# iammcy/BFLC-demo

Measured on NVIDIA H100. Metric: federated_rounds_per_sec, higher is better.
Workload: dtype mxfp8

## Files before the change

bflc_demo_b200/csrc/kernels/mlp_round_sm100.cu:

```cuda
#include <cuda_bf16.h>

#include <algorithm>
#include <cstdlib>
#include <cstring>
#include <type_traits>

#include "bflc_kernels.h"
#include "epi_common.cuh"
#include "fed_admit.cuh"
#include "launch.cuh"
#include "sm100_ptx.cuh"
#include "wgmma.cuh"

namespace bflc {

namespace {

using epi::kStgLd;
using epi::stage_put;
using epi::stage_get;
using epi::col_sum32;
using epi::st_sw128;
__device__ __forceinline__ uint32_t pack2(float a, float b) { return epi::pack_bf16x2(a, b); }

constexpr int kBM = 128, kBN = 64, kStages = 5;
constexpr int kABytes = kBM * 128, kBBytes = kBN * 128, kStageBytes = kABytes + kBBytes;
constexpr int kTileBytes = kStages * kStageBytes;
constexpr int kBarBytes = 512;
constexpr int kEpiWarps = 8;
constexpr int kEpiThreads = kEpiWarps * 32;
constexpr int kStgAll = kEpiWarps * 32 * kStgLd * 4;
constexpr int kBiasFloats = 320;
constexpr int kXchFloats = 4 * 2 * 128;
constexpr int kAccPitch = kBN + 4;
constexpr int kAccBytes = kBM * kAccPitch * 4;
constexpr int kSmemTotal = kTileBytes + kBarBytes + kStgAll + (kBiasFloats + kXchFloats) * 4 + kAccBytes + 1024;
static_assert(kSmemTotal <= 227 * 1024, "shared memory budget");
constexpr int kEpiT0 = 128;
constexpr int kProducerWarp = 4 + kEpiWarps;
constexpr int kThreads = kEpiT0 + kEpiThreads + 128;
constexpr int kProducerRegs = 40, kMmaRegs = 184, kEpiRegs = 144;
static_assert(kProducerRegs + kMmaRegs + 2 * kEpiRegs <= 4 * 128, "register file");
enum Role : int { kRoleProducer = 0, kRoleMma = 1, kRoleEpi = 2 };
constexpr int kGrid = 32;

constexpr int kOffH = 0;
constexpr int kOffW2K = 64 * 1024;
constexpr int kOffW2MN = 96 * 1024;
constexpr int kOffDL = 104 * 1024;
static_assert(kOffDL + 16384 <= kTileBytes, "chain smem layout");
constexpr int kChainH = 256;
constexpr int kDefaultPlan = 4;
constexpr int kCluster = 4;

enum EpiMode : int { E_BIAS_RELU_BF16 = 0, E_XENT = 1, E_F32 = 2, E_MASK_COLSUM_BF16 = 3,
                     E_OPT = 4 };

struct Maps {
  CUtensorMap x_k, w1_k, h_k, w2_k, dl_mn, h_mn, dl_k, w2_mn, dh_mn, x_mn;
};

struct Args {
  int B, steps, in_dim, hidden, n_classes, ncp;
  int chain;
  int epiopt;
  unsigned long long* dbg;
  const unsigned int* x_ready;
  const unsigned int* round_seq;
// ... 82 lines not shown
}

__device__ __forceinline__ void produce_tile(const Job& j, uint8_t* smem, uint64_t* full_bar, uint64_t* empty_bar,
                                             Pipe& pp) {
  const uint32_t a_bytes = static_cast<uint32_t>(j.bm) * 128u;
  for (int i = 0; i < j.n_kb; ++i, ++pp.it) {
    const int s = pp.it % kStages;
    const uint32_t ph = (pp.it / kStages) & 1;
    ptx::mbar_wait(&empty_bar[s], ph ^ 1);
    uint8_t* sa = smem + s * kStageBytes;
    uint8_t* sb = sa + kABytes;
    if (ptx::elect_one()) {
      ptx::mbar_expect_tx(&full_bar[s], a_bytes + kBBytes);
      if (!j.a_mn) {
        ptx::tma_load_3d(sa, j.ta, &full_bar[s], j.a_c0 + i * 64, j.a_c1, 0);
      } else {
        ptx::tma_load_3d(sa, j.ta, &full_bar[s], j.a_c0, j.a_c1 + i * 64, 0);
        if (j.bm == kBM) ptx::tma_load_3d(sa + 64 * 128, j.ta, &full_bar[s], j.a_c0 + 64, j.a_c1 + i * 64, 0);
      }
      if (!j.b_mn)
        ptx::tma_load_3d(sb, j.tb, &full_bar[s], j.b_c0 + i * 64, j.b_c1, 0);
      else
        ptx::tma_load_3d(sb, j.tb, &full_bar[s], j.b_c0, j.b_c1 + i * 64, 0);
    }
    __syncwarp();
  }
}

__device__ __forceinline__ int lane128(int r) { return r; }
__device__ __forceinline__ int lane128_hi(int r) { return 64 + r; }
// ... 364 lines not shown
  }
  if (stampit) j.dbg[j.dbg_slot + 1] = globaltimer_ns();
}

__device__ __forceinline__ uint32_t pos_mask8(const uint4 u) {
  const uint32_t wds[4] = {u.x, u.y, u.z, u.w};
  uint32_t m = 0u;
#pragma unroll
  for (int e = 0; e < 4; ++e) {
    m |= (((wds[e] & 0xFFFFu) != 0u && (wds[e] & 0x8000u) == 0u) ? 1u : 0u) << (e * 2);
    m |= (((wds[e] >> 16) != 0u && (wds[e] & 0x80000000u) == 0u) ? 1u : 0u) << (e * 2 + 1);
  }
  return m;
}

template <bool FP8>
__device__ __forceinline__ uint32_t fwd1_epilogue_x(const Job& j, const Args& a, uint8_t* smem, const ChainBars& cb,
                                                    int q, int half, int lane, uint64_t* accum_bar,
                                                    const wg::AccTile& at, float* stg, float* sbias, Pipe& pp,
                                                    uint32_t par, int slice) {
  const int et = threadIdx.x - kEpiT0;
  if (et < kBN) sbias[et] = __ldcg(j.bias + j.n0 + et);
  epi_bar();
  const int rl = q * 32 + lane, row_base = j.m0 + q * 32;
  const bool row_ok = row_base + lane < j.M;
  const int cr = lane >> 3, cg = (lane & 7) * 4, nc = j.n0 + half * 32;
  const bool stampit = j.dbg != nullptr && blockIdx.x == 0 && threadIdx.x == kEpiT0;
  ptx::mbar_wait(accum_bar, pp.tile & 1);
  ++pp.tile;
  if (stampit) j.dbg[j.dbg_slot] = globaltimer_ns();
  float v[32];
  {
    uint32_t r[32];
    wg::acc_ld32(at, (static_cast<uint32_t>(q * 32) << 16) + half * 32, r);
#pragma unroll
    for (int k = 0; k < 32; ++k) v[k] = fmaxf(__uint_as_float(r[k]) + sbias[half * 32 + k], 0.f);
  }
  uint4 hv[4];
  if (FP8) {
    uint32_t w[8];
    const int e = epi::mx8_quant32(v, w);
#pragma unroll
    for (int i = 0; i < 4; ++i) {
      const uint2 lo = epi::mx8_dq4(w[2 * i], e), hi = epi::mx8_dq4(w[2 * i + 1], e);
      hv[i] = make_uint4(lo.x, lo.y, hi.x, hi.y);
    }
  } else {
#pragma unroll
    for (int jj = 0; jj < 4; ++jj)
      hv[jj] = make_uint4(pack2(v[8 * jj], v[8 * jj + 1]), pack2(v[8 * jj + 2], v[8 * jj + 3]),
                          pack2(v[8 * jj + 4], v[8 * jj + 5]), pack2(v[8 * jj + 6], v[8 * jj + 7]));
  }
  uint32_t mk = 0u;
#pragma unroll
  for (int jj = 0; jj < 4; ++jj) {
    if (!row_ok) hv[jj] = make_uint4(0u, 0u, 0u, 0u);
    mk |= pos_mask8(hv[jj]) << (jj * 8);
  }
  stage_put(stg, lane, v);
  uint8_t* hs = smem + kOffH + slice * 16384;
#pragma unroll
  for (int jj = 0; jj < 4; ++jj) st_sw128(hs, rl, half * 4 + jj, hv[jj]);
  ptx::fence_proxy_async_smem();
  epi_bar();
  if (threadIdx.x == kEpiT0) {
    const uint32_t hxa = ptx::smem_u32(cb.hx);
    ptx::mbar_expect_tx(cb.hx, (kCluster - 1) * 16384);
    ptx::mbar_wait_cluster(cb.ring_free, par);
    for (uint32_t r = 1; r < kCluster; ++r) {
      const uint32_t peer = (slice + r) % kCluster;
      ptx::bulk_s2cluster(ptx::mapa(ptx::smem_u32(hs), peer), hs, 16384, ptx::mapa(hxa, peer));
    }
  }
  if (stampit) j.dbg[1] = globaltimer_ns();
  __syncwarp();
#pragma unroll
  for (int it = 0; it < 8; ++it) {
    const int rr = it * 4 + cr, rw = row_base + rr;
    if (rw >= j.M) continue;
    const float4 x = *reinterpret_cast<const float4*>(stg + rr * kStgLd + cg);
    *reinterpret_cast<uint2*>(a.h + static_cast<long long>(rw) * j.ldd + nc + cg) =
        make_uint2(pack2(x.x, x.y), pack2(x.z, x.w));
  }
  __syncwarp();
  if (stampit) j.dbg[j.dbg_slot + 1] = globaltimer_ns();
  return mk;
}

__device__ __forceinline__ void chain_produce(const Maps& maps, uint8_t* smem, const ChainBars& cb, int m0,
                                              int slice, bool with_h) {
  if (ptx::elect_one()) {
    ptx::mbar_expect_tx(cb.w2k, 32768);
    if (with_h) ptx::mbar_expect_tx(cb.h, 65536);
    ptx::mbar_expect_tx(cb.w2mn, 8192);
    if (with_h) {
#pragma unroll
      for (int kb = 0; kb < 4; ++kb)
        ptx::tma_load_3d(smem + kOffH + kb * 16384, &maps.h_k, cb.h, kb * 64, m0, 0);
    }
#pragma unroll
    for (int kb = 0; kb < 4; ++kb)
      ptx::tma_load_3d(smem + kOffW2K + kb * 8192, &maps.w2_k, cb.w2k, kb * 64, 0, 0);
    ptx::tma_load_3d(smem + kOffW2MN, &maps.w2_mn, cb.w2mn, slice * 64, 0, 0);
  }
  __syncwarp();
}

__device__ __forceinline__ void chain_mma(uint8_t* smem, const ChainBars& cb, const wg::AccTile& at, uint32_t par,
                                          bool fused) {
  const uint32_t base = ptx::smem_u32(smem);
  ptx::mbar_wait(cb.w2k, par);
  if (fused) {
    ptx::mbar_wait_cluster(cb.hx, par);
    ptx::fence_proxy_async_smem();
  } else {
    ptx::mbar_wait(cb.h, par);
  }
  float l0[32], l1[32];
  wg::zero(l0);
  wg::zero(l1);
  const uint32_t ha = base + kOffH, wb = base + kOffW2K;
  wg::fence();
#pragma unroll
  for (uint32_t kb = 0; kb < 4; ++kb)
#pragma unroll
    for (uint32_t k = 0; k < 4; ++k) {
      const uint64_t bd = wg::desc(wb + kb * 8192u + k * 32u, 16);
      wg::mma_bf16<64, 0, 0>(l0, wg::desc(ha + kb * 16384u + k * 32u, 16), bd, (kb > 0 || k > 0) ? 1u : 0u);
      wg::mma_bf16<64, 0, 0>(l1, wg::desc(ha + kb * 16384u + 8192u + k * 32u, 16), bd, (kb > 0 || k > 0) ? 1u : 0u);
    }
  wg::commit();
  wg::wait<0>();
  wg::reg_fence(l0);
  wg::reg_fence(l1);
  wg::acc_put<64>(at, 0, l0, lane128);
  wg::acc_put<64>(at, 0, l1, lane128_hi);
  ptx::mbar_arrive(cb.acc_l);
  ptx::mbar_wait(cb.w2mn, par);
  ptx::mbar_wait(cb.dl_ready, par);
  wg::zero(l0);
  wg::zero(l1);
  wg::fence();
#pragma unroll
  for (uint32_t k = 0; k < 4; ++k) {
    const uint64_t bd = wg::desc(base + kOffW2MN + k * 2048u, 8192);
    wg::mma_bf16<64, 0, 1>(l0, wg::desc(base + kOffDL + k * 32u, 16), bd, k > 0);
    wg::mma_bf16<64, 0, 1>(l1, wg::desc(base + kOffDL + 8192u + k * 32u, 16), bd, k > 0);
  }
  wg::commit();
  wg::wait<0>();
  wg::reg_fence(l0);
  wg::reg_fence(l1);
  wg::acc_put<64>(at, 0, l0, lane128);
  wg::acc_put<64>(at, 0, l1, lane128_hi);
  ptx::mbar_arrive(cb.acc_dh);
}

__device__ __forceinline__ void chain_epilogue(const Args& a, uint8_t* smem, const ChainBars& cb,
                                               const wg::AccTile& at, int q, int half, int lane, float* stg,
                                               float* sb, float* xch, uint32_t par, int m0, int r0, int slice,
                                               unsigned long long* dbg, bool fused, uint32_t mk_fused) {
  auto stampc = [&](int slot) {
    if (dbg != nullptr && blockIdx.x == 0 && threadIdx.x == kEpiT0) dbg[slot] = globaltimer_ns();
  };
  const int rl = q * 32 + lane;
  const int row = m0 + rl;
  const bool row_ok = row < a.B;
  const int32_t label = row_ok ? __ldg(a.labels + r0 + row) : -1;
  const int C = a.n_classes;
  {
    const int et = threadIdx.x - kEpiT0;
    sb[et] = __ldcg(a.b1 + et);
    if (et < 64) sb[kChainH + et] = et < C ? __ldcg(a.b2 + et) : 0.f;
    epi_bar();
  }
  const uint32_t taddr = static_cast<uint32_t>(q * 32) << 16;
  float* xmax = xch + half * 128;            const float* omax = xch + (1 - half) * 128;
  float* xidx = xch + 256 + half * 128;      const float* oidx = xch + 256 + (1 - half) * 128;
  float* xzl = xch + 512 + half * 128;       const float* ozl = xch + 512 + (1 - half) * 128;
  float* xsum = xch + 768 + half * 128;      const float* osum = xch + 768 + (1 - half) * 128;

  uint32_t mk = mk_fused;
  if (!fused) {
    ptx::mbar_wait(cb.h, par);
    stampc(6);
    const uint8_t* hs = smem + kOffH;
    const int c = 2 * slice + half;
#pragma unroll
    for (int jj = 0; jj < 4; ++jj) mk |= pos_mask8(epi::ld_sw128(hs + (c >> 1) * 16384, rl, (c & 1) * 4 + jj)) << (jj * 8);
  } else if (dbg != nullptr && blockIdx.x == 0 && threadIdx.x == kEpiT0) {
    ptx::mbar_wait_cluster(cb.hx, par);
    stampc(6);
  }
  stampc(7);

  ptx::mbar_wait(cb.acc_l, par);
  stampc(8);
  {
    float z[32];
    {
      uint32_t ra[32];
      wg::acc_ld32(at, taddr + half * 32, ra);
#pragma unroll
      for (int k = 0; k < 32; ++k) z[k] = __uint_as_float(ra[k]) + sb[kChainH + half * 32 + k];
    }
    const int nb = half * 32;
    float pm[4] = {-INFINITY, -INFINITY, -INFINITY, -INFINITY};
    int pi[4] = {-1, -1, -1, -1};
    float zlab = 0.f;
#pragma unroll
    for (int k = 0; k < 32; ++k) {
      if (nb + k < C) {
        if (z[k] > pm[k & 3]) { pm[k & 3] = z[k]; pi[k & 3] = nb + k; }
        if (nb + k == label) zlab = z[k];
      }
    }
    float vmax = pm[0];
    int amax = pi[0];
#pragma unroll
    for (int jq = 1; jq < 4; ++jq)
      if (pm[jq] > vmax || (pm[jq] == vmax && pi[jq] >= 0 && pi[jq] < amax)) { vmax = pm[jq]; amax = pi[jq]; }
    xmax[rl] = vmax; xidx[rl] = __int_as_float(amax); xzl[rl] = zlab;
    epi_bar();
    {
      const float ov = omax[rl];
      const int oi = __float_as_int(oidx[rl]);
      const bool take = half == 0 ? (ov > vmax) : (ov >= vmax && oi >= 0);
      if (take) { vmax = ov; amax = oi; }
      zlab += ozl[rl];
    }
    stampc(12);
    float ps[4] = {0.f, 0.f, 0.f, 0.f};
#pragma unroll
    for (int k = 0; k < 32; ++k) {
      z[k] = nb + k < C ? __expf(z[k] - vmax) : 0.f;
      ps[k & 3] += z[k];
    }
    const float psum = (ps[0] + ps[1]) + (ps[2] + ps[3]);
    xsum[rl] = psum;
    epi_bar();
    const float sum = psum + osum[rl];
    const float inv = 1.f / sum;
    const float gs = 1.f / static_cast<float>(a.B);
    const bool do_colsum = slice == 1, do_global = slice == 2, do_loss = slice == 3 && half == 0;
    uint8_t* dls = smem + kOffDL;
    {
      float v[32];
#pragma unroll
      for (int k = 0; k < 32; ++k)
        v[k] = (nb + k < C && row_ok) ? (z[k] * inv - (nb + k == label ? 1.f : 0.f)) * gs : 0.f;
#pragma unroll
      for (int jj = 0; jj < 4; ++jj) {
        const uint4 u = make_uint4(pack2(v[8 * jj], v[8 * jj + 1]), pack2(v[8 * jj + 2], v[8 * jj + 3]),
                                   pack2(v[8 * jj + 4], v[8 * jj + 5]), pack2(v[8 * jj + 6], v[8 * jj + 7]));
        st_sw128(dls, rl, half * 4 + jj, u);
      }
      if (do_colsum) {
        stage_put(stg, lane, v);
        __syncwarp();
        const float tot = col_sum32(stg, lane, 32);
        if (nb + lane < C) atomicAdd(a.gb2 + nb + lane, tot);
        __syncwarp();
      }
    }
    stampc(13);
    ptx::fence_proxy_async_smem();
    ptx::mbar_arrive(cb.dl_ready);
    stampc(14);
    __syncwarp();
    if (do_global) {
#pragma unroll
      for (int it = 0; it < 4; ++it) {
        const int rt = q * 32 + it * 8 + (lane >> 2), ch = half * 4 + (lane & 3);
        const uint4 u = epi::ld_sw128(dls, rt, ch);
        if (m0 + rt < a.B && ch * 8 < a.ncp)
          *reinterpret_cast<uint4*>(a.dlogits + static_cast<long long>(m0 + rt) * a.ncp + ch * 8) = u;
      }
    }
    if (do_loss) {
      float loss = row_ok ? (__logf(sum) + vmax - zlab) : 0.f;
      const bool hit = row_ok && (amax == label);
#pragma unroll
      for (int off = 16; off >= 1; off >>= 1) loss += __shfl_xor_sync(0xffffffffu, loss, off);
      const unsigned cnt = __popc(__ballot_sync(0xffffffffu, hit));
      if (lane == 0) {
        atomicAdd(a.loss_sum, loss);
        if (cnt) atomicAdd(a.correct, cnt);
      }
    }
  }
  stampc(9);

  ptx::mbar_wait(cb.acc_dh, par);
  stampc(10);
  {
    uint8_t* ds = smem + kOffH + (fused ? ((slice + 1) % kCluster) * 16384 : 0);
    uint32_t r[32];
    wg::acc_ld32(at, taddr + half * 32, r);
    float v[32];
#pragma unroll
    for (int k = 0; k < 32; ++k) v[k] = ((mk >> k) & 1u) ? __uint_as_float(r[k]) : 0.f;
#pragma unroll
    for (int jj = 0; jj < 4; ++jj)
      st_sw128(ds, rl, half * 4 + jj,
               make_uint4(pack2(v[8 * jj], v[8 * jj + 1]), pack2(v[8 * jj + 2], v[8 * jj + 3]),
                          pack2(v[8 * jj + 4], v[8 * jj + 5]), pack2(v[8 * jj + 6], v[8 * jj + 7])));
    stage_put(stg, lane, v);
    __syncwarp();
    const float tot = col_sum32(stg, lane, 32);
    atomicAdd(a.gb1 + (2 * slice + half) * 32 + lane, tot);
#pragma unroll
    for (int it = 0; it < 4; ++it) {
      const int rt = q * 32 + it * 8 + (lane >> 2), ch = half * 4 + (lane & 3);
      const uint4 u = epi::ld_sw128(ds, rt, ch);
      if (m0 + rt < a.B)
        *reinterpret_cast<uint4*>(a.dh + static_cast<long long>(m0 + rt) * a.hidden + slice * 64 + ch * 8) = u;
    }
    __syncwarp();
  }
  stampc(11);
}

__device__ __forceinline__ void grid_barrier(unsigned int* counter, unsigned int& epoch, bool sys = false) {
  ++epoch;
  __syncthreads();
  if (threadIdx.x == 0) {
    ptx::fence_proxy_async_all();
    if (sys) __threadfence_system(); else __threadfence();
    atomicAdd(counter, 1u);
    const unsigned int target = epoch * gridDim.x;
    unsigned long long spins = 0;
    while (true) {
      unsigned int v;
// ... 7 lines not shown
}

template <bool FP8>
__global__ void __launch_bounds__(kThreads, 1)
mlp_round_kernel(const __grid_constant__ Maps maps, const Args a) {
  extern __shared__ uint8_t smem_raw[];
  uint8_t* smem = reinterpret_cast<uint8_t*>(
      (reinterpret_cast<uintptr_t>(smem_raw) + 1023) & ~static_cast<uintptr_t>(1023));
  uint64_t* full_bar = reinterpret_cast<uint64_t*>(smem + kTileBytes);
  uint64_t* empty_bar = full_bar + kStages;
  uint64_t* accum_bar = empty_bar + kStages;
  uint64_t* cbar = accum_bar + 1;
  ChainBars cb{cbar, cbar + 1, cbar + 2, cbar + 3, cbar + 4, cbar + 5, cbar + 6, cbar + 7};
  float* stage_base = reinterpret_cast<float*>(smem + kTileBytes + kBarBytes);
  float* sbias = stage_base + kEpiWarps * 32 * kStgLd;
  float* xch = sbias + kBiasFloats;
  const wg::AccTile at{xch + kXchFloats, kAccPitch};

  ptx::pdl_launch_dependents();
  const int warp = threadIdx.x >> 5, lane = threadIdx.x & 31;
  __shared__ int ticket;

  auto role_body = [&](auto role_tag) __attribute__((always_inline)) {
  constexpr int ROLE = decltype(role_tag)::value;
  if (warp == 0 && lane == 0) {
    for (int s = 0; s < kStages; ++s) {
      ptx::mbar_init(&full_bar[s], 1);
      ptx::mbar_init(&empty_bar[s], 128);
    }
    ptx::mbar_init(accum_bar, 128);
    ptx::mbar_init(cb.h, 1); ptx::mbar_init(cb.w2k, 1); ptx::mbar_init(cb.w2mn, 1);
    ptx::mbar_init(cb.acc_l, 128); ptx::mbar_init(cb.acc_dh, 128);
// ... 9 lines not shown

  Pipe pp{0u, 0u};
  uint32_t chains = 0;
  bool x_all_ready = false;
  unsigned int bar_epoch = 0;
  const int t = blockIdx.x;
  const int q = warp & 3, half = (warp - 4) >> 2;
  float* stg = stage_base + (warp >= 4 && warp < kProducerWarp ? warp - 4 : 0) * (32 * kStgLd);
  const int B = a.B, H = a.hidden, C = a.n_classes, D = a.in_dim;
  const int mt_b = (B + kBM - 1) / kBM;
  const int nt_h = (H + kBN - 1) / kBN;
  const int nt_d = (D + kBN - 1) / kBN;
  const int bm_w = a.bm_w;
  const int mt_hw = (H + bm_w - 1) / bm_w;
  const int kb_d = (D + 63) / 64, kb_h = (H + 63) / 64, kb_b = (B + 63) / 64, kb_c = (C + 63) / 64;
  const int p1_tiles = mt_b * nt_h;
  const bool fused = a.chain == 4;
  uint32_t mk = 0u;

  auto run = [&](const Job& j) {
    if constexpr (ROLE == kRoleEpi) epilogue_tile<FP8>(j, a, q, half, lane, accum_bar, at, stg, sbias, pp);
    else if constexpr (ROLE == kRoleMma) mma_tile(j, smem, full_bar, empty_bar, accum_bar, at, pp);
    else if (warp == kProducerWarp) produce_tile(j, smem, full_bar, empty_bar, pp);
  };

  auto stamp = [&](int step, int slot) {
    if (a.dbg != nullptr && blockIdx.x == 0 && threadIdx.x == kEpiT0) a.dbg[step * 32 + slot] = globaltimer_ns();
  };
  for (int step = 0; step < a.steps; ++step) {
    const int r0 = step * B;
    const bool last = step == a.steps - 1;
    float bc1 = 1.f, bc2 = 1.f;
// ... 13 lines not shown
          unsigned int v;
          asm volatile("ld.acquire.gpu.global.u32 %0, [%1];" : "=r"(v) : "l"(a.x_ready + a.steps - 1) : "memory");
          all = static_cast<int>(v - want) >= 0 ? 1 : 0;
          unsigned long long spins = 0;
          while (!all) {
            asm volatile("ld.acquire.gpu.global.u32 %0, [%1];" : "=r"(v) : "l"(a.x_ready + step) : "memory");
            if (static_cast<int>(v - want) >= 0) break;
            if (++spins > (1ull << 28)) __trap();
            __nanosleep(32);
          }
        }
        x_all_ready = __shfl_sync(0xffffffffu, all, 0) != 0;
        ptx::fence_proxy_async_all();
      }
      Job j{};
      j.mode = E_BIAS_RELU_BF16; j.d = a.h; j.ldd = H; j.bias = a.b1; j.M = B; j.N = H; j.bm = kBM;
      j.dbg = sdbg; j.dbg_slot = 16;
      j.m0 = (t / nt_h) * kBM; j.n0 = (t % nt_h) * kBN;
      j.ta = &maps.x_k; j.tb = &maps.w1_k; j.a_mn = 0; j.b_mn = 0;
      j.a_c0 = 0; j.a_c1 = r0 + j.m0; j.b_c0 = 0; j.b_c1 = j.n0; j.n_kb = kb_d;
      if (!fused) {
        run(j);
      } else {
        const uint32_t par = chains & 1;
        if constexpr (ROLE == kRoleEpi) {
          mk = fwd1_epilogue_x<FP8>(j, a, smem, cb, q, half, lane, accum_bar, at, stg, sbias, pp, par, t % 4);
        } else if constexpr (ROLE == kRoleMma) {
          mma_tile(j, smem, full_bar, empty_bar, accum_bar, at, pp, cb.ring_free);
        } else if (warp == kProducerWarp) {
          produce_tile(j, smem, full_bar, empty_bar, pp);
          const uint32_t last = pp.it - 1;
          ptx::mbar_wait(&empty_bar[last % kStages], (last / kStages) & 1);
          chain_produce(maps, smem, cb, j.m0, t % 4, false);
        }
      }
    }
    if (!fused) {
      grid_barrier(a.barrier, bar_epoch);
      stamp(step, 1);
    }
    if (a.chain != 0) {
      if (t < mt_b * 4) {
        const int m0 = (t / 4) * kBM, slice = t % 4;
        const uint32_t par = chains & 1;
        if constexpr (ROLE == kRoleEpi)
          chain_epilogue(a, smem, cb, at, q, half, lane, stg, sbias, xch, par, m0, r0, slice, sdbg, fused, mk);
        else if constexpr (ROLE == kRoleMma) chain_mma(smem, cb, at, par, fused);
        else if (warp == kProducerWarp && !fused) chain_produce(maps, smem, cb, m0, slice, true);
        ++chains;
      }
      grid_barrier(a.barrier, bar_epoch);
      stamp(step, 2);
    } else {
      if (t < mt_b) {
        Job j{};
        j.ta = &maps.h_k; j.tb = &maps.w2_k; j.a_mn = 0; j.b_mn = 0; j.bm = kBM;
        j.m0 = t * kBM; j.n0 = 0; j.M = B; j.N = C;
        j.a_c0 = 0; j.a_c1 = j.m0; j.b_c0 = 0; j.b_c1 = 0; j.n_kb = kb_h;
        j.mode = E_XENT; j.d = a.dlogits; j.ldd = a.ncp; j.bias = a.b2; j.colsum = a.gb2;
        j.labels = a.labels + r0; j.grad_scale = 1.f / static_cast<float>(B);
        run(j);
      }
      grid_barrier(a.barrier, bar_epoch);
// ... 153 lines not shown
  const bool epiopt = r.epiopt >= 0 ? r.epiopt != 0 : epiopt_env0;
  const bool chain_ok = r.hidden == kChainH && r.ncp == 64 && r.n_classes <= 64;
  int chain = (!chain_ok || chain_env == 0) ? 0 : chain_env == 4 ? 4 : 3;
  const bool fp8 = r.fp8;
  if (fp8 && (chain == 0 || !epiopt || r.batch % 128 || r.in_dim % 16 || !r.x_dq || !r.work_q || !r.work_dq ||
              !r.h_dq))
    return cudaErrorNotSupported;
  if (r.fed != nullptr && !epiopt) return cudaErrorNotSupported;
  static const int bmw_env = [] { const char* e = std::getenv("BFLC_MLP_BMW"); return e && std::atoi(e) == 128 ? 128 : 64; }();
  int bm_w = bmw_env;
  int mt_hw = (r.hidden + bm_w - 1) / bm_w;
  int dev = 0, sms = 0;
  if (cudaGetDevice(&dev) != cudaSuccess || cudaDeviceGetAttribute(&sms, cudaDevAttrMultiProcessorCount, dev) != cudaSuccess)
    return cudaErrorInvalidDevice;
  if (mt_hw * nt_d + nt_h + 1 > sms) { bm_w = 128; mt_hw = (r.hidden + 127) / 128; }
  const int need = std::max(std::max(mt_b * nt_h, mt_hw * nt_d + nt_h + 1), chain != 0 ? mt_b * 4 : 0);
  int grid = need > kGrid ? need : kGrid;
  if (grid > sms) return cudaErrorInvalidValue;

  static bool configured[2] = {false, false};
  if (!configured[fp8 ? 1 : 0]) {
    const cudaError_t ea =
        fp8 ? cudaFuncSetAttribute(mlp_round_kernel<true>, cudaFuncAttributeMaxDynamicSharedMemorySize, kSmemTotal)
            : cudaFuncSetAttribute(mlp_round_kernel<false>, cudaFuncAttributeMaxDynamicSharedMemorySize, kSmemTotal);
    if (ea != cudaSuccess) return ea;
    configured[fp8 ? 1 : 0] = true;
  }
  if (chain == 4) {
    static int max_clusters[2] = {-1, -1};
    int& mc = max_clusters[fp8 ? 1 : 0];
    const int grid4 = (grid + kCluster - 1) / kCluster * kCluster;
    if (mc < 0) {
      cudaLaunchConfig_t cfg{};
      cudaLaunchAttribute attr[1];
      attr[0].id = cudaLaunchAttributeClusterDimension;
      attr[0].val.clusterDim.x = kCluster; attr[0].val.clusterDim.y = 1; attr[0].val.clusterDim.z = 1;
      cfg.gridDim = dim3(grid4);
      cfg.blockDim = dim3(kThreads);
      cfg.dynamicSmemBytes = kSmemTotal;
      cfg.attrs = attr;
      cfg.numAttrs = 1;
      int n = 0;
      const cudaError_t eo = fp8 ? cudaOccupancyMaxActiveClusters(&n, mlp_round_kernel<true>, &cfg)
                                 : cudaOccupancyMaxActiveClusters(&n, mlp_round_kernel<false>, &cfg);
      if (eo != cudaSuccess) { (void)cudaGetLastError(); n = 0; }
      mc = n;
    }
    if (grid4 <= sms && mc * kCluster >= grid4) grid = grid4;
    else chain = 3;
  }

  Maps m;
  std::memset(&m, 0, sizeof(m));
  const long long rows_x = static_cast<long long>(r.steps) * r.batch;
  auto mk = [&](CUtensorMap* out, const void* ptr, long long ld, bool mn, int rows_extent, int K,
                int rows_tile, DType dt = DType::BF16) {
    GemmOperand op{ptr, ld, 0, mn};
    return gemm_make_operand_map(out, op, dt, rows_extent, K, 1, rows_tile);
  };
  cudaError_t e;
  const void* fx = fp8 ? r.x_dq : r.x;
  const void* fw1 = fp8 ? static_cast<const void*>(r.work_dq) : r.w1_shadow;
  const void* fh = fp8 ? r.h_dq : r.h;
  const void* fw2 = fp8 ? static_cast<const void*>(r.work_dq + static_cast<long long>(r.hidden) * r.in_dim)
                        : r.w2_shadow;
  if ((e = mk(&m.x_k, fx, r.in_dim, false, (int)rows_x, r.in_dim, kBM)) != cudaSuccess) return e;
  if ((e = mk(&m.w1_k, fw1, r.in_dim, false, r.hidden, r.in_dim, kBN)) != cudaSuccess) return e;
  if ((e = mk(&m.h_k, fh, r.hidden, false, r.batch, r.hidden, kBM)) != cudaSuccess) return e;
  if ((e = mk(&m.w2_k, fw2, r.hidden, false, r.n_classes, r.hidden, kBN)) != cudaSuccess) return e;
  if ((e = mk(&m.dl_mn, r.dlogits, r.ncp, true, r.n_classes, r.batch, kBM)) != cudaSuccess) return e;
  if ((e = mk(&m.h_mn, r.h, r.hidden, true, r.hidden, r.batch, kBN)) != cudaSuccess) return e;
  if ((e = mk(&m.dl_k, r.dlogits, r.ncp, false, r.batch, r.n_classes, kBM)) != cudaSuccess) return e;
  if ((e = mk(&m.w2_mn, r.w2_shadow, r.hidden, true, r.hidden, r.n_classes, kBN)) != cudaSuccess) return e;
  if ((e = mk(&m.dh_mn, r.dh, r.hidden, true, r.hidden, r.batch, kBM)) != cudaSuccess) return e;
  if ((e = mk(&m.x_mn, r.x, r.in_dim, true, r.in_dim, (int)rows_x, kBN)) != cudaSuccess) return e;
  const Mx8MlpLayout ql = mx8_mlp_layout(r.in_dim, r.hidden);

  Args a{};
  a.B = r.batch; a.steps = r.steps; a.in_dim = r.in_dim; a.hidden = r.hidden;
  a.n_classes = r.n_classes; a.ncp = r.ncp; a.n_params = r.n_params;
  a.chain = chain; a.epiopt = epiopt ? 1 : 0; a.dbg = r.dbg;
  a.x_ready = r.x_ready; a.round_seq = r.round_seq;
  a.pred = r.pred ? r.pred : current_predicate();
  a.barrier = r.barrier;
  a.master = r.master; a.b1 = r.b1; a.b2 = r.b2;
  a.grad = r.grad; a.gw1 = r.gw1; a.gb1 = r.gb1; a.gw2 = r.gw2; a.gb2 = r.gb2;
  a.shadow = reinterpret_cast<__nv_bfloat16*>(r.shadow);
// ... 22 lines not shown
```

Before: 3691.

## Use 64-row tiles in fused cluster chain to spread batch over more CTAs

In the fused cluster chain mode, the first forward GEMM and the chain epilogue/MMA now use 64-row M tiles instead of 128. This doubles the number of row tiles and CTAs working on the batch. The epilogues are rewritten to read the accumulator directly from smem with per-thread row/column ownership. Cross-half exchange buffers are replaced by warp shuffles, and the bias-gradient column sum moves to a shared reduction tile. TMA boxes are narrowed to 64 rows, with two loads issued for 128-row tiles. The grid sizing now depends on chain mode and falls back when clusters do not fit, at the cost of more smaller MMAs and more atomics.

```diff
diff --git a/bflc_demo_b200/csrc/kernels/mlp_round_sm100.cu b/bflc_demo_b200/csrc/kernels/mlp_round_sm100.cu
--- a/bflc_demo_b200/csrc/kernels/mlp_round_sm100.cu
+++ b/bflc_demo_b200/csrc/kernels/mlp_round_sm100.cu
@@ -31,10 +31,11 @@
 constexpr int kEpiThreads = kEpiWarps * 32;
 constexpr int kStgAll = kEpiWarps * 32 * kStgLd * 4;
 constexpr int kBiasFloats = 320;
-constexpr int kXchFloats = 4 * 2 * 128;
 constexpr int kAccPitch = kBN + 4;
 constexpr int kAccBytes = kBM * kAccPitch * 4;
-constexpr int kSmemTotal = kTileBytes + kBarBytes + kStgAll + (kBiasFloats + kXchFloats) * 4 + kAccBytes + 1024;
+constexpr int kRedLd = kBN + 4;
+static_assert(kBM * kRedLd * 4 <= kStgAll, "column-sum tile");
+constexpr int kSmemTotal = kTileBytes + kBarBytes + kStgAll + kBiasFloats * 4 + kAccBytes + 1024;
 static_assert(kSmemTotal <= 227 * 1024, "shared memory budget");
 constexpr int kEpiT0 = 128;
 constexpr int kProducerWarp = 4 + kEpiWarps;
@@ -52,6 +53,8 @@
 constexpr int kChainH = 256;
 constexpr int kDefaultPlan = 4;
 constexpr int kCluster = 4;
+constexpr int kBMx = 64;
+constexpr int kHSlice = kBMx * 128;
 
 enum EpiMode : int { E_BIAS_RELU_BF16 = 0, E_XENT = 1, E_F32 = 2, E_MASK_COLSUM_BF16 = 3,
                      E_OPT = 4 };
@@ -164,6 +167,7 @@
       ptx::mbar_expect_tx(&full_bar[s], a_bytes + kBBytes);
       if (!j.a_mn) {
         ptx::tma_load_3d(sa, j.ta, &full_bar[s], j.a_c0 + i * 64, j.a_c1, 0);
+        if (j.bm == kBM) ptx::tma_load_3d(sa + 64 * 128, j.ta, &full_bar[s], j.a_c0 + i * 64, j.a_c1 + 64, 0);
       } else {
         ptx::tma_load_3d(sa, j.ta, &full_bar[s], j.a_c0, j.a_c1 + i * 64, 0);
         if (j.bm == kBM) ptx::tma_load_3d(sa + 64 * 128, j.ta, &full_bar[s], j.a_c0 + 64, j.a_c1 + i * 64, 0);
@@ -558,75 +562,99 @@
   return m;
 }
 
+template <int BM>
+struct ChainThread {
+  static constexpr int kRpw = BM / 8, kTpr = 32 / kRpw, kCpt = 64 / kTpr;
+  int rl, c;
+  const float* acc;
+  __device__ __forceinline__ ChainThread(const wg::AccTile& at, int lane) {
+    rl = kRpw * ((static_cast<int>(threadIdx.x) - kEpiT0) >> 5) + lane % kRpw;
+    c = lane / kRpw;
+    acc = at.p + (BM == 64 ? lane64(rl) : lane128(rl)) * at.pitch;
+  }
+};
+
+template <int BM>
+__device__ __forceinline__ void red_colsum(const float* red, float* dst, int n) {
+  epi_bar();
+  const int et = threadIdx.x - kEpiT0, col = et & 63, r0 = (et >> 6) * 32;
+  if (r0 >= BM) return;
+  float t[4] = {0.f, 0.f, 0.f, 0.f};
+#pragma unroll
+  for (int rr = 0; rr < 32; ++rr) t[rr & 3] += red[(r0 + rr) * kRedLd + col];
+  if (col < n) atomicAdd(dst + col, (t[0] + t[1]) + (t[2] + t[3]));
+}
+
 template <bool FP8>
 __device__ __forceinline__ uint32_t fwd1_epilogue_x(const Job& j, const Args& a, uint8_t* smem, const ChainBars& cb,
-                                                    int q, int half, int lane, uint64_t* accum_bar,
-                                                    const wg::AccTile& at, float* stg, float* sbias, Pipe& pp,
-                                                    uint32_t par, int slice) {
+                                                    int lane, uint64_t* accum_bar, const wg::AccTile& at,
+                                                    float* sbias, Pipe& pp, uint32_t par, int slice) {
   const int et = threadIdx.x - kEpiT0;
   if (et < kBN) sbias[et] = __ldcg(j.bias + j.n0 + et);
   epi_bar();
-  const int rl = q * 32 + lane, row_base = j.m0 + q * 32;
-  const bool row_ok = row_base + lane < j.M;
-  const int cr = lane >> 3, cg = (lane & 7) * 4, nc = j.n0 + half * 32;
+  const ChainThread<kBMx> th(at, lane);
+  const int row = j.m0 + th.rl, c0 = th.c * 16;
+  const bool row_ok = row < j.M;
   const bool stampit = j.dbg != nullptr && blockIdx.x == 0 && threadIdx.x == kEpiT0;
   ptx::mbar_wait(accum_bar, pp.tile & 1);
   ++pp.tile;
   if (stampit) j.dbg[j.dbg_slot] = globaltimer_ns();
-  float v[32];
-  {
-    uint32_t r[32];
-    wg::acc_ld32(at, (static_cast<uint32_t>(q * 32) << 16) + half * 32, r);
-#pragma unroll
-    for (int k = 0; k < 32; ++k) v[k] = fmaxf(__uint_as_float(r[k]) + sbias[half * 32 + k], 0.f);
-  }
-  uint4 hv[4];
+  float v[16];
+#pragma unroll
+  for (int k = 0; k < 4; ++k) {
+    const float4 t = reinterpret_cast<const float4*>(th.acc + c0)[k];
+    v[4 * k] = fmaxf(t.x + sbias[c0 + 4 * k], 0.f);
+    v[4 * k + 1] = fmaxf(t.y + sbias[c0 + 4 * k + 1], 0.f);
+    v[4 * k + 2] = fmaxf(t.z + sbias[c0 + 4 * k + 2], 0.f);
+    v[4 * k + 3] = fmaxf(t.w + sbias[c0 + 4 * k + 3], 0.f);
+  }
+  uint4 hb[2];
+#pragma unroll
+  for (int jj = 0; jj < 2; ++jj)
+    hb[jj] = make_uint4(pack2(v[8 * jj], v[8 * jj + 1]), pack2(v[8 * jj + 2], v[8 * jj + 3]),
+                        pack2(v[8 * jj + 4], v[8 * jj + 5]), pack2(v[8 * jj + 6], v[8 * jj + 7]));
+  uint4 hv[2] = {hb[0], hb[1]};
   if (FP8) {
-    uint32_t w[8];
-    const int e = epi::mx8_quant32(v, w);
-#pragma unroll
-    for (int i = 0; i < 4; ++i) {
-      const uint2 lo = epi::mx8_dq4(w[2 * i], e), hi = epi::mx8_dq4(w[2 * i + 1], e);
-      hv[i] = make_uint4(lo.x, lo.y, hi.x, hi.y);
-    }
-  } else {
-#pragma unroll
-    for (int jj = 0; jj < 4; ++jj)
-      hv[jj] = make_uint4(pack2(v[8 * jj], v[8 * jj + 1]), pack2(v[8 * jj + 2], v[8 * jj + 3]),
-                          pack2(v[8 * jj + 4], v[8 * jj + 5]), pack2(v[8 * jj + 6], v[8 * jj + 7]));
+    float amax = 0.f;
+#pragma unroll
+    for (int k = 0; k < 16; ++k) amax = fmaxf(amax, fabsf(v[k]));
+    amax = fmaxf(amax, __shfl_xor_sync(0xffffffffu, amax, 8));
+    const int e = epi::mx8_scale_byte(amax);
+    const float inv = epi::mx8_inv_scale(e);
+#pragma unroll
+    for (int jj = 0; jj < 2; ++jj) {
+      const float* x = v + 8 * jj;
+      const uint2 lo = epi::mx8_dq4(epi::mx8_pack4(x[0] * inv, x[1] * inv, x[2] * inv, x[3] * inv), e);
+      const uint2 hi = epi::mx8_dq4(epi::mx8_pack4(x[4] * inv, x[5] * inv, x[6] * inv, x[7] * inv), e);
+      hv[jj] = make_uint4(lo.x, lo.y, hi.x, hi.y);
+    }
   }
   uint32_t mk = 0u;
 #pragma unroll
-  for (int jj = 0; jj < 4; ++jj) {
+  for (int jj = 0; jj < 2; ++jj) {
     if (!row_ok) hv[jj] = make_uint4(0u, 0u, 0u, 0u);
     mk |= pos_mask8(hv[jj]) << (jj * 8);
   }
-  stage_put(stg, lane, v);
-  uint8_t* hs = smem + kOffH + slice * 16384;
-#pragma unroll
-  for (int jj = 0; jj < 4; ++jj) st_sw128(hs, rl, half * 4 + jj, hv[jj]);
+  uint8_t* hs = smem + kOffH + slice * kHSlice;
+#pragma unroll
+  for (int jj = 0; jj < 2; ++jj) st_sw128(hs, th.rl, 2 * th.c + jj, hv[jj]);
   ptx::fence_proxy_async_smem();
   epi_bar();
   if (threadIdx.x == kEpiT0) {
     const uint32_t hxa = ptx::smem_u32(cb.hx);
-    ptx::mbar_expect_tx(cb.hx, (kCluster - 1) * 16384);
+    ptx::mbar_expect_tx(cb.hx, (kCluster - 1) * kHSlice);
     ptx::mbar_wait_cluster(cb.ring_free, par);
     for (uint32_t r = 1; r < kCluster; ++r) {
       const uint32_t peer = (slice + r) % kCluster;
-      ptx::bulk_s2cluster(ptx::mapa(ptx::smem_u32(hs), peer), hs, 16384, ptx::mapa(hxa, peer));
+      ptx::bulk_s2cluster(ptx::mapa(ptx::smem_u32(hs), peer), hs, kHSlice, ptx::mapa(hxa, peer));
     }
   }
   if (stampit) j.dbg[1] = globaltimer_ns();
-  __syncwarp();
-#pragma unroll
-  for (int it = 0; it < 8; ++it) {
-    const int rr = it * 4 + cr, rw = row_base + rr;
-    if (rw >= j.M) continue;
-    const float4 x = *reinterpret_cast<const float4*>(stg + rr * kStgLd + cg);
-    *reinterpret_cast<uint2*>(a.h + static_cast<long long>(rw) * j.ldd + nc + cg) =
-        make_uint2(pack2(x.x, x.y), pack2(x.z, x.w));
-  }
-  __syncwarp();
+  if (row_ok) {
+    uint4* d = reinterpret_cast<uint4*>(a.h + static_cast<long long>(row) * j.ldd + j.n0 + c0);
+    d[0] = hb[0];
+    d[1] = hb[1];
+  }
   if (stampit) j.dbg[j.dbg_slot + 1] = globaltimer_ns();
   return mk;
 }
@@ -639,8 +667,10 @@
     ptx::mbar_expect_tx(cb.w2mn, 8192);
     if (with_h) {
 #pragma unroll
-      for (int kb = 0; kb < 4; ++kb)
+      for (int kb = 0; kb < 4; ++kb) {
         ptx::tma_load_3d(smem + kOffH + kb * 16384, &maps.h_k, cb.h, kb * 64, m0, 0);
+        ptx::tma_load_3d(smem + kOffH + kb * 16384 + 8192, &maps.h_k, cb.h, kb * 64, m0 + 64, 0);
+      }
     }
 #pragma unroll
     for (int kb = 0; kb < 4; ++kb)
@@ -650,8 +680,11 @@
   __syncwarp();
 }
 
+template <int BM>
 __device__ __forceinline__ void chain_mma(uint8_t* smem, const ChainBars& cb, const wg::AccTile& at, uint32_t par,
                                           bool fused) {
+  constexpr bool two = BM == kBM;
+  constexpr uint32_t kb_bytes = BM * 128u;
   const uint32_t base = ptx::smem_u32(smem);
   ptx::mbar_wait(cb.w2k, par);
   if (fused) {
@@ -670,15 +703,20 @@
 #pragma unroll
     for (uint32_t k = 0; k < 4; ++k) {
       const uint64_t bd = wg::desc(wb + kb * 8192u + k * 32u, 16);
-      wg::mma_bf16<64, 0, 0>(l0, wg::desc(ha + kb * 16384u + k * 32u, 16), bd, (kb > 0 || k > 0) ? 1u : 0u);
-      wg::mma_bf16<64, 0, 0>(l1, wg::desc(ha + kb * 16384u + 8192u + k * 32u, 16), bd, (kb > 0 || k > 0) ? 1u : 0u);
+      wg::mma_bf16<64, 0, 0>(l0, wg::desc(ha + kb * kb_bytes + k * 32u, 16), bd, (kb > 0 || k > 0) ? 1u : 0u);
+      if (two)
+        wg::mma_bf16<64, 0, 0>(l1, wg::desc(ha + kb * kb_bytes + 8192u + k * 32u, 16), bd, (kb > 0 || k > 0) ? 1u : 0u);
     }
   wg::commit();
   wg::wait<0>();
   wg::reg_fence(l0);
-  wg::reg_fence(l1);
-  wg::acc_put<64>(at, 0, l0, lane128);
-  wg::acc_put<64>(at, 0, l1, lane128_hi);
+  if (two) {
+    wg::reg_fence(l1);
+    wg::acc_put<64>(at, 0, l0, lane128);
+    wg::acc_put<64>(at, 0, l1, lane128_hi);
+  } else {
+    wg::acc_put<64>(at, 0, l0, lane64);
+  }
   ptx::mbar_arrive(cb.acc_l);
   ptx::mbar_wait(cb.w2mn, par);
   ptx::mbar_wait(cb.dl_ready, par);
@@ -689,49 +727,53 @@
   for (uint32_t k = 0; k < 4; ++k) {
     const uint64_t bd = wg::desc(base + kOffW2MN + k * 2048u, 8192);
     wg::mma_bf16<64, 0, 1>(l0, wg::desc(base + kOffDL + k * 32u, 16), bd, k > 0);
-    wg::mma_bf16<64, 0, 1>(l1, wg::desc(base + kOffDL + 8192u + k * 32u, 16), bd, k > 0);
+    if (two) wg::mma_bf16<64, 0, 1>(l1, wg::desc(base + kOffDL + 8192u + k * 32u, 16), bd, k > 0);
   }
   wg::commit();
   wg::wait<0>();
   wg::reg_fence(l0);
-  wg::reg_fence(l1);
-  wg::acc_put<64>(at, 0, l0, lane128);
-  wg::acc_put<64>(at, 0, l1, lane128_hi);
+  if (two) {
+    wg::reg_fence(l1);
+    wg::acc_put<64>(at, 0, l0, lane128);
+    wg::acc_put<64>(at, 0, l1, lane128_hi);
+  } else {
+    wg::acc_put<64>(at, 0, l0, lane64);
+  }
   ptx::mbar_arrive(cb.acc_dh);
 }
 
+template <int BM>
 __device__ __forceinline__ void chain_epilogue(const Args& a, uint8_t* smem, const ChainBars& cb,
-                                               const wg::AccTile& at, int q, int half, int lane, float* stg,
-                                               float* sb, float* xch, uint32_t par, int m0, int r0, int slice,
+                                               const wg::AccTile& at, int lane, float* red, float* sb,
+                                               uint32_t par, int m0, int r0, int slice,
                                                unsigned long long* dbg, bool fused, uint32_t mk_fused) {
+  using TH = ChainThread<BM>;
+  constexpr int kTpr = TH::kTpr, kCpt = TH::kCpt;
   auto stampc = [&](int slot) {
     if (dbg != nullptr && blockIdx.x == 0 && threadIdx.x == kEpiT0) dbg[slot] = globaltimer_ns();
   };
-  const int rl = q * 32 + lane;
+  const TH th(at, lane);
+  const int rl = th.rl;
   const int row = m0 + rl;
   const bool row_ok = row < a.B;
   const int32_t label = row_ok ? __ldg(a.labels + r0 + row) : -1;
   const int C = a.n_classes;
+  const int et = threadIdx.x - kEpiT0;
   {
-    const int et = threadIdx.x - kEpiT0;
     sb[et] = __ldcg(a.b1 + et);
     if (et < 64) sb[kChainH + et] = et < C ? __ldcg(a.b2 + et) : 0.f;
     epi_bar();
   }
-  const uint32_t taddr = static_cast<uint32_t>(q * 32) << 16;
-  float* xmax = xch + half * 128;            const float* omax = xch + (1 - half) * 128;
-  float* xidx = xch + 256 + half * 128;      const float* oidx = xch + 256 + (1 - half) * 128;
-  float* xzl = xch + 512 + half * 128;       const float* ozl = xch + 512 + (1 - half) * 128;
-  float* xsum = xch + 768 + half * 128;      const float* osum = xch + 768 + (1 - half) * 128;
+  const int rw0 = TH::kRpw * (et >> 5);
 
   uint32_t mk = mk_fused;
   if (!fused) {
     ptx::mbar_wait(cb.h, par);
     stampc(6);
-    const uint8_t* hs = smem + kOffH;
-    const int c = 2 * slice + half;
-#pragma unroll
-    for (int jj = 0; jj < 4; ++jj) mk |= pos_mask8(epi::ld_sw128(hs + (c >> 1) * 16384, rl, (c & 1) * 4 + jj)) << (jj * 8);
+    const uint8_t* hs = smem + kOffH + slice * (BM * 128);
+#pragma unroll
+    for (int jj = 0; jj < kCpt / 8; ++jj)
+      mk |= pos_mask8(epi::ld_sw128(hs, rl, th.c * (kCpt / 8) + jj)) << (jj * 8);
   } else if (dbg != nullptr && blockIdx.x == 0 && threadIdx.x == kEpiT0) {
     ptx::mbar_wait_cluster(cb.hx, par);
     stampc(6);
@@ -741,89 +783,104 @@
   ptx::mbar_wait(cb.acc_l, par);
   stampc(8);
   {
-    float z[32];
-    {
-      uint32_t ra[32];
-      wg::acc_ld32(at, taddr + half * 32, ra);
-#pragma unroll
-      for (int k = 0; k < 32; ++k) z[k] = __uint_as_float(ra[k]) + sb[kChainH + half * 32 + k];
-    }
-    const int nb = half * 32;
-    float pm[4] = {-INFINITY, -INFINITY, -INFINITY, -INFINITY};
-    int pi[4] = {-1, -1, -1, -1};
-    float zlab = 0.f;
-#pragma unroll
-    for (int k = 0; k < 32; ++k) {
-      if (nb + k < C) {
-        if (z[k] > pm[k & 3]) { pm[k & 3] = z[k]; pi[k & 3] = nb + k; }
-        if (nb + k == label) zlab = z[k];
-      }
-    }
-    float vmax = pm[0];
-    int amax = pi[0];
-#pragma unroll
-    for (int jq = 1; jq < 4; ++jq)
-      if (pm[jq] > vmax || (pm[jq] == vmax && pi[jq] >= 0 && pi[jq] < amax)) { vmax = pm[jq]; amax = pi[jq]; }
-    xmax[rl] = vmax; xidx[rl] = __int_as_float(amax); xzl[rl] = zlab;
-    epi_bar();
-    {
-      const float ov = omax[rl];
-      const int oi = __float_as_int(oidx[rl]);
-      const bool take = half == 0 ? (ov > vmax) : (ov >= vmax && oi >= 0);
-      if (take) { vmax = ov; amax = oi; }
-      zlab += ozl[rl];
+    constexpr int NJ = 8 / kTpr;
+    const int hh = th.c / (kTpr / 2), j0 = (th.c % (kTpr / 2)) * NJ;
+    const int nb = 32 * hh + j0;
+    float z[8 * NJ];
+#pragma unroll
+    for (int i = 0; i < 8; ++i) {
+      const float* src = th.acc + nb + 4 * i;
+      if constexpr (NJ == 4) {
+        const float4 t = *reinterpret_cast<const float4*>(src);
+        z[4 * i] = t.x; z[4 * i + 1] = t.y; z[4 * i + 2] = t.z; z[4 * i + 3] = t.w;
+      } else {
+        const float2 t = *reinterpret_cast<const float2*>(src);
+        z[2 * i] = t.x; z[2 * i + 1] = t.y;
+      }
+#pragma unroll
+      for (int jj = 0; jj < NJ; ++jj) z[NJ * i + jj] += sb[kChainH + nb + 4 * i + jj];
+    }
+    float vmax = -INFINITY, zlab = 0.f;
+    int amax = -1;
+#pragma unroll
+    for (int i = 0; i < 8; ++i)
+#pragma unroll
+      for (int jj = 0; jj < NJ; ++jj) {
+        const int n = nb + 4 * i + jj;
+        const float x = z[NJ * i + jj];
+        if (n < C) {
+          if (x > vmax) { vmax = x; amax = n; }
+          if (n == label) zlab = x;
+        }
+      }
+#pragma unroll
+    for (int off = (kTpr == 4 ? 8 : 16); off <= 16; off <<= 1) {
+      const float ov = __shfl_xor_sync(0xffffffffu, vmax, off);
+      const int oi = __shfl_xor_sync(0xffffffffu, amax, off);
+      if (ov > vmax || (ov == vmax && oi >= 0 && (amax < 0 || oi < amax))) { vmax = ov; amax = oi; }
+      zlab += __shfl_xor_sync(0xffffffffu, zlab, off);
     }
     stampc(12);
-    float ps[4] = {0.f, 0.f, 0.f, 0.f};
-#pragma unroll
-    for (int k = 0; k < 32; ++k) {
-      z[k] = nb + k < C ? __expf(z[k] - vmax) : 0.f;
-      ps[k & 3] += z[k];
-    }
-    const float psum = (ps[0] + ps[1]) + (ps[2] + ps[3]);
-    xsum[rl] = psum;
-    epi_bar();
-    const float sum = psum + osum[rl];
+    float ps[NJ];
+#pragma unroll
+    for (int jj = 0; jj < NJ; ++jj) ps[jj] = 0.f;
+#pragma unroll
+    for (int i = 0; i < 8; ++i)
+#pragma unroll
+      for (int jj = 0; jj < NJ; ++jj) {
+        float& x = z[NJ * i + jj];
+        x = nb + 4 * i + jj < C ? __expf(x - vmax) : 0.f;
+        ps[jj] += x;
+      }
+    float psum;
+    if constexpr (NJ == 4) {
+      psum = (ps[0] + ps[1]) + (ps[2] + ps[3]);
+    } else {
+      psum = ps[0] + ps[1];
+      psum += __shfl_xor_sync(0xffffffffu, psum, 8);
+    }
+    const float sum = psum + __shfl_xor_sync(0xffffffffu, psum, 16);
     const float inv = 1.f / sum;
     const float gs = 1.f / static_cast<float>(a.B);
-    const bool do_colsum = slice == 1, do_global = slice == 2, do_loss = slice == 3 && half == 0;
+    const bool do_colsum = slice == 1, do_global = slice == 2, do_loss = slice == 3;
     uint8_t* dls = smem + kOffDL;
-    {
-      float v[32];
-#pragma unroll
-      for (int k = 0; k < 32; ++k)
-        v[k] = (nb + k < C && row_ok) ? (z[k] * inv - (nb + k == label ? 1.f : 0.f)) * gs : 0.f;
-#pragma unroll
-      for (int jj = 0; jj < 4; ++jj) {
-        const uint4 u = make_uint4(pack2(v[8 * jj], v[8 * jj + 1]), pack2(v[8 * jj + 2], v[8 * jj + 3]),
-                                   pack2(v[8 * jj + 4], v[8 * jj + 5]), pack2(v[8 * jj + 6], v[8 * jj + 7]));
-        st_sw128(dls, rl, half * 4 + jj, u);
-      }
-      if (do_colsum) {
-        stage_put(stg, lane, v);
-        __syncwarp();
-        const float tot = col_sum32(stg, lane, 32);
-        if (nb + lane < C) atomicAdd(a.gb2 + nb + lane, tot);
-        __syncwarp();
+#pragma unroll
+    for (int i = 0; i < 8; ++i) {
+      float v[NJ];
+#pragma unroll
+      for (int jj = 0; jj < NJ; ++jj) {
+        const int n = nb + 4 * i + jj;
+        v[jj] = (n < C && row_ok) ? (z[NJ * i + jj] * inv - (n == label ? 1.f : 0.f)) * gs : 0.f;
+      }
+      const int col = nb + 4 * i;
+      uint8_t* d = dls + rl * 128 + (((col >> 3) ^ (rl & 7)) << 4) + (col & 7) * 2;
+      if constexpr (NJ == 4) {
+        *reinterpret_cast<uint2*>(d) = make_uint2(pack2(v[0], v[1]), pack2(v[2], v[3]));
+        if (do_colsum) *reinterpret_cast<float4*>(red + rl * kRedLd + col) = make_float4(v[0], v[1], v[2], v[3]);
+      } else {
+        *reinterpret_cast<uint32_t*>(d) = pack2(v[0], v[1]);
+        if (do_colsum) *reinterpret_cast<float2*>(red + rl * kRedLd + col) = make_float2(v[0], v[1]);
       }
     }
     stampc(13);
     ptx::fence_proxy_async_smem();
     ptx::mbar_arrive(cb.dl_ready);
     stampc(14);
+    if (do_colsum) red_colsum<BM>(red, a.gb2, C);
     __syncwarp();
     if (do_global) {
 #pragma unroll
-      for (int it = 0; it < 4; ++it) {
-        const int rt = q * 32 + it * 8 + (lane >> 2), ch = half * 4 + (lane & 3);
+      for (int it = 0; it < TH::kRpw / 4; ++it) {
+        const int rt = rw0 + 4 * it + (lane >> 3), ch = lane & 7;
         const uint4 u = epi::ld_sw128(dls, rt, ch);
         if (m0 + rt < a.B && ch * 8 < a.ncp)
           *reinterpret_cast<uint4*>(a.dlogits + static_cast<long long>(m0 + rt) * a.ncp + ch * 8) = u;
       }
     }
     if (do_loss) {
-      float loss = row_ok ? (__logf(sum) + vmax - zlab) : 0.f;
-      const bool hit = row_ok && (amax == label);
+      const bool own = th.c == 0 && row_ok;
+      float loss = own ? (__logf(sum) + vmax - zlab) : 0.f;
+      const bool hit = own && (amax == label);
 #pragma unroll
       for (int off = 16; off >= 1; off >>= 1) loss += __shfl_xor_sync(0xffffffffu, loss, off);
       const unsigned cnt = __popc(__ballot_sync(0xffffffffu, hit));
@@ -832,35 +889,40 @@
         if (cnt) atomicAdd(a.correct, cnt);
       }
     }
+    if (do_colsum) epi_bar();
   }
   stampc(9);
 
   ptx::mbar_wait(cb.acc_dh, par);
   stampc(10);
   {
-    uint8_t* ds = smem + kOffH + (fused ? ((slice + 1) % kCluster) * 16384 : 0);
-    uint32_t r[32];
-    wg::acc_ld32(at, taddr + half * 32, r);
-    float v[32];
-#pragma unroll
-    for (int k = 0; k < 32; ++k) v[k] = ((mk >> k) & 1u) ? __uint_as_float(r[k]) : 0.f;
-#pragma unroll
-    for (int jj = 0; jj < 4; ++jj)
-      st_sw128(ds, rl, half * 4 + jj,
-               make_uint4(pack2(v[8 * jj], v[8 * jj + 1]), pack2(v[8 * jj + 2], v[8 * jj + 3]),
-                          pack2(v[8 * jj + 4], v[8 * jj + 5]), pack2(v[8 * jj + 6], v[8 * jj + 7])));
-    stage_put(stg, lane, v);
-    __syncwarp();
-    const float tot = col_sum32(stg, lane, 32);
-    atomicAdd(a.gb1 + (2 * slice + half) * 32 + lane, tot);
-#pragma unroll
-    for (int it = 0; it < 4; ++it) {
-      const int rt = q * 32 + it * 8 + (lane >> 2), ch = half * 4 + (lane & 3);
+    uint8_t* ds = smem + kOffH + (fused ? ((slice + 1) % kCluster) * kHSlice : 0);
+    const int c0 = th.c * kCpt;
+#pragma unroll
+    for (int jj = 0; jj < kCpt / 8; ++jj) {
+      float v[8];
+#pragma unroll
+      for (int h2 = 0; h2 < 2; ++h2) {
+        const float4 t = *reinterpret_cast<const float4*>(th.acc + c0 + 8 * jj + 4 * h2);
+        const int b = 8 * jj + 4 * h2;
+        v[4 * h2] = ((mk >> b) & 1u) ? t.x : 0.f;
+        v[4 * h2 + 1] = ((mk >> (b + 1)) & 1u) ? t.y : 0.f;
+        v[4 * h2 + 2] = ((mk >> (b + 2)) & 1u) ? t.z : 0.f;
+        v[4 * h2 + 3] = ((mk >> (b + 3)) & 1u) ? t.w : 0.f;
+        *reinterpret_cast<float4*>(red + rl * kRedLd + c0 + b) = make_float4(v[4 * h2], v[4 * h2 + 1],
+                                                                             v[4 * h2 + 2], v[4 * h2 + 3]);
+      }
+      st_sw128(ds, rl, th.c * (kCpt / 8) + jj,
+               make_uint4(pack2(v[0], v[1]), pack2(v[2], v[3]), pack2(v[4], v[5]), pack2(v[6], v[7])));
+    }
+    red_colsum<BM>(red, a.gb1 + slice * 64, 64);
+#pragma unroll
+    for (int it = 0; it < TH::kRpw / 4; ++it) {
+      const int rt = rw0 + 4 * it + (lane >> 3), ch = lane & 7;
       const uint4 u = epi::ld_sw128(ds, rt, ch);
       if (m0 + rt < a.B)
         *reinterpret_cast<uint4*>(a.dh + static_cast<long long>(m0 + rt) * a.hidden + slice * 64 + ch * 8) = u;
     }
-    __syncwarp();
   }
   stampc(11);
 }
@@ -898,8 +960,7 @@
   ChainBars cb{cbar, cbar + 1, cbar + 2, cbar + 3, cbar + 4, cbar + 5, cbar + 6, cbar + 7};
   float* stage_base = reinterpret_cast<float*>(smem + kTileBytes + kBarBytes);
   float* sbias = stage_base + kEpiWarps * 32 * kStgLd;
-  float* xch = sbias + kBiasFloats;
-  const wg::AccTile at{xch + kXchFloats, kAccPitch};
+  const wg::AccTile at{sbias + kBiasFloats, kAccPitch};
 
   ptx::pdl_launch_dependents();
   const int warp = threadIdx.x >> 5, lane = threadIdx.x & 31;
@@ -939,8 +1000,10 @@
   const int bm_w = a.bm_w;
   const int mt_hw = (H + bm_w - 1) / bm_w;
   const int kb_d = (D + 63) / 64, kb_h = (H + 63) / 64, kb_b = (B + 63) / 64, kb_c = (C + 63) / 64;
-  const int p1_tiles = mt_b * nt_h;
   const bool fused = a.chain == 4;
+  const int bm_x = fused ? kBMx : kBM;
+  const int mt_x = (B + bm_x - 1) / bm_x;
+  const int p1_tiles = mt_x * nt_h;
   uint32_t mk = 0u;
 
   auto run = [&](const Job& j) {
@@ -984,9 +1047,9 @@
         ptx::fence_proxy_async_all();
       }
       Job j{};
-      j.mode = E_BIAS_RELU_BF16; j.d = a.h; j.ldd = H; j.bias = a.b1; j.M = B; j.N = H; j.bm = kBM;
+      j.mode = E_BIAS_RELU_BF16; j.d = a.h; j.ldd = H; j.bias = a.b1; j.M = B; j.N = H; j.bm = bm_x;
       j.dbg = sdbg; j.dbg_slot = 16;
-      j.m0 = (t / nt_h) * kBM; j.n0 = (t % nt_h) * kBN;
+      j.m0 = (t / nt_h) * bm_x; j.n0 = (t % nt_h) * kBN;
       j.ta = &maps.x_k; j.tb = &maps.w1_k; j.a_mn = 0; j.b_mn = 0;
       j.a_c0 = 0; j.a_c1 = r0 + j.m0; j.b_c0 = 0; j.b_c1 = j.n0; j.n_kb = kb_d;
       if (!fused) {
@@ -994,7 +1057,7 @@
       } else {
         const uint32_t par = chains & 1;
         if constexpr (ROLE == kRoleEpi) {
-          mk = fwd1_epilogue_x<FP8>(j, a, smem, cb, q, half, lane, accum_bar, at, stg, sbias, pp, par, t % 4);
+          mk = fwd1_epilogue_x<FP8>(j, a, smem, cb, lane, accum_bar, at, sbias, pp, par, t % 4);
         } else if constexpr (ROLE == kRoleMma) {
           mma_tile(j, smem, full_bar, empty_bar, accum_bar, at, pp, cb.ring_free);
         } else if (warp == kProducerWarp) {
@@ -1010,13 +1073,16 @@
       stamp(step, 1);
     }
     if (a.chain != 0) {
-      if (t < mt_b * 4) {
-        const int m0 = (t / 4) * kBM, slice = t % 4;
+      if (t < mt_x * 4) {
+        const int m0 = (t / 4) * bm_x, slice = t % 4;
         const uint32_t par = chains & 1;
-        if constexpr (ROLE == kRoleEpi)
-          chain_epilogue(a, smem, cb, at, q, half, lane, stg, sbias, xch, par, m0, r0, slice, sdbg, fused, mk);
-        else if constexpr (ROLE == kRoleMma) chain_mma(smem, cb, at, par, fused);
-        else if (warp == kProducerWarp && !fused) chain_produce(maps, smem, cb, m0, slice, true);
+        if constexpr (ROLE == kRoleEpi) {
+          if (fused) chain_epilogue<kBMx>(a, smem, cb, at, lane, stage_base, sbias, par, m0, r0, slice, sdbg, true, mk);
+          else chain_epilogue<kBM>(a, smem, cb, at, lane, stage_base, sbias, par, m0, r0, slice, sdbg, false, 0u);
+        } else if constexpr (ROLE == kRoleMma) {
+          if (fused) chain_mma<kBMx>(smem, cb, at, par, true);
+          else chain_mma<kBM>(smem, cb, at, par, false);
+        } else if (warp == kProducerWarp && !fused) chain_produce(maps, smem, cb, m0, slice, true);
         ++chains;
       }
       grid_barrier(a.barrier, bar_epoch);
@@ -1200,9 +1266,12 @@
   if (cudaGetDevice(&dev) != cudaSuccess || cudaDeviceGetAttribute(&sms, cudaDevAttrMultiProcessorCount, dev) != cudaSuccess)
     return cudaErrorInvalidDevice;
   if (mt_hw * nt_d + nt_h + 1 > sms) { bm_w = 128; mt_hw = (r.hidden + 127) / 128; }
-  const int need = std::max(std::max(mt_b * nt_h, mt_hw * nt_d + nt_h + 1), chain != 0 ? mt_b * 4 : 0);
-  int grid = need > kGrid ? need : kGrid;
-  if (grid > sms) return cudaErrorInvalidValue;
+  auto need = [&](int ch) {
+    const int mt_x = ch == 4 ? (r.batch + kBMx - 1) / kBMx : mt_b;
+    return std::max({mt_x * nt_h, mt_hw * nt_d + nt_h + 1, ch != 0 ? mt_x * 4 : 0, kGrid});
+  };
+  int grid = need(chain);
+  if (chain != 4 && grid > sms) return cudaErrorInvalidValue;
 
   static bool configured[2] = {false, false};
   if (!configured[fp8 ? 1 : 0]) {
@@ -1232,8 +1301,13 @@
       if (eo != cudaSuccess) { (void)cudaGetLastError(); n = 0; }
       mc = n;
     }
-    if (grid4 <= sms && mc * kCluster >= grid4) grid = grid4;
-    else chain = 3;
+    if (grid4 <= sms && mc * kCluster >= grid4) {
+      grid = grid4;
+    } else {
+      chain = 3;
+      grid = need(3);
+      if (grid > sms) return cudaErrorInvalidValue;
+    }
   }
 
   Maps m;
@@ -1250,13 +1324,13 @@
   const void* fh = fp8 ? r.h_dq : r.h;
   const void* fw2 = fp8 ? static_cast<const void*>(r.work_dq + static_cast<long long>(r.hidden) * r.in_dim)
                         : r.w2_shadow;
-  if ((e = mk(&m.x_k, fx, r.in_dim, false, (int)rows_x, r.in_dim, kBM)) != cudaSuccess) return e;
+  if ((e = mk(&m.x_k, fx, r.in_dim, false, (int)rows_x, r.in_dim, 64)) != cudaSuccess) return e;
   if ((e = mk(&m.w1_k, fw1, r.in_dim, false, r.hidden, r.in_dim, kBN)) != cudaSuccess) return e;
-  if ((e = mk(&m.h_k, fh, r.hidden, false, r.batch, r.hidden, kBM)) != cudaSuccess) return e;
+  if ((e = mk(&m.h_k, fh, r.hidden, false, r.batch, r.hidden, 64)) != cudaSuccess) return e;
   if ((e = mk(&m.w2_k, fw2, r.hidden, false, r.n_classes, r.hidden, kBN)) != cudaSuccess) return e;
   if ((e = mk(&m.dl_mn, r.dlogits, r.ncp, true, r.n_classes, r.batch, kBM)) != cudaSuccess) return e;
   if ((e = mk(&m.h_mn, r.h, r.hidden, true, r.hidden, r.batch, kBN)) != cudaSuccess) return e;
-  if ((e = mk(&m.dl_k, r.dlogits, r.ncp, false, r.batch, r.n_classes, kBM)) != cudaSuccess) return e;
+  if ((e = mk(&m.dl_k, r.dlogits, r.ncp, false, r.batch, r.n_classes, 64)) != cudaSuccess) return e;
   if ((e = mk(&m.w2_mn, r.w2_shadow, r.hidden, true, r.hidden, r.n_classes, kBN)) != cudaSuccess) return e;
   if ((e = mk(&m.dh_mn, r.dh, r.hidden, true, r.hidden, r.batch, kBM)) != cudaSuccess) return e;
   if ((e = mk(&m.x_mn, r.x, r.in_dim, true, r.in_dim, (int)rows_x, kBN)) != cudaSuccess) return e;
```

Result: faster. 4100, median of 6 (+11.1%).
